# Patman86/SVT-AV1-Mod-by-Patman

Measured on AMD Instinct MI355X. Metric: encoded fps (4K 10-bit preset 8) + ME+txfm HBM GB/s vs roofline, 1/2/4/8 GPU, higher is better.
Workload: dtype u8 (ME) / int32 (transform)

## Files before the change

include/svt_hip_me.h:

```cpp
#ifndef SVT_HIP_ME_H
#define SVT_HIP_ME_H

#include "svt_hip.h"

#ifdef __cplusplus
extern "C" {
#endif

SVT_HIP_API void svt_sad_loop_kernel_hip(uint8_t *src, uint32_t src_stride, uint8_t *ref,
                                         uint32_t ref_stride, uint32_t block_height,
                                         uint32_t block_width, uint64_t *best_sad,
                                         int16_t *x_search_center, int16_t *y_search_center,
                                         uint32_t src_stride_raw, uint8_t skip_search_line,
                                         int16_t search_area_width, int16_t search_area_height);

SVT_HIP_API uint32_t svt_nxm_sad_kernel_hip(const uint8_t *src, uint32_t src_stride,
                                            const uint8_t *ref, uint32_t ref_stride,
                                            uint32_t height, uint32_t width);

SVT_HIP_API uint32_t svt_nxm_sad_kernel_sub_sampled_hip(const uint8_t *src, uint32_t src_stride,
                                                        const uint8_t *ref, uint32_t ref_stride,
                                                        uint32_t height, uint32_t width);
SVT_HIP_API uint32_t svt_aom_sad_16b_kernel_hip(uint16_t *src, uint32_t src_stride, uint16_t *ref,
                                                uint32_t ref_stride, uint32_t height, uint32_t width);
// ... 147 lines not shown
    uint64_t hme_sad;
    int16_t  hme_sc_x, hme_sc_y;
    uint8_t  do_ref;
    uint8_t  pad_[3];
} SvtHipMeSearchResult;

typedef struct SvtHipMeFrameOut {
    uint32_t *best_sad;
    uint32_t *best_mv;
    SvtHipMeSearchResult *search_results;
    uint32_t *me_mv_array;
    uint8_t  *me_candidate_array;
    uint8_t  *total_me_candidate_index;
    uint32_t *me_64x64_distortion, *me_32x32_distortion, *me_16x16_distortion, *me_8x8_distortion;
    uint32_t *me_8x8_cost_variance;
    uint32_t *rc_me_distortion;
} SvtHipMeFrameOut;

typedef struct SvtHipMeFrameJob {
    SvtHipMeParams   prm;
    SvtHipPyramid8   src;
    SvtHipPyramid8   ref[SVT_HIP_ME_MAX_LIST][SVT_HIP_ME_MAX_REF];
    SvtHipMeFrameOut out;
} SvtHipMeFrameJob;

SVT_HIP_API uint32_t svt_hip_me_b64_count(uint32_t width, uint32_t height);

SVT_HIP_API int32_t svt_hip_me_frames(const SvtHipMeFrameJob *jobs, uint32_t n_jobs, void *stream);

SVT_HIP_API int32_t svt_hip_me_validate_jobs(const SvtHipMeFrameJob *jobs, uint32_t n_jobs, uint32_t *max_b64);
SVT_HIP_API int32_t svt_hip_me_frames_dev(const SvtHipMeFrameJob *d_jobs, uint32_t n_jobs, uint32_t max_b64,
                                          void *stream);

typedef enum SvtHipRtcdSlot {
    SVT_HIP_SLOT_SAD_LOOP_KERNEL = 0,
    SVT_HIP_SLOT_NXM_SAD_KERNEL,
    SVT_HIP_SLOT_EXT_ALL_SAD_8X8_16X16,
    SVT_HIP_SLOT_EXT_EIGHT_SAD_32X32_64X64,
    SVT_HIP_SLOT_EXT_SAD_8X8_16X16,
    SVT_HIP_SLOT_EXT_SAD_32X32_64X64,
    SVT_HIP_SLOT_DOWNSAMPLE_2D,
    SVT_HIP_SLOT_COMPUTE_INTERM_VAR_FOUR8X8,
    SVT_HIP_SLOT_COMPUTE_SUB_MEAN_8X8,
    SVT_HIP_SLOT_COMPUTE_MEAN_8X8,
    SVT_HIP_SLOT_COMPUTE_MEAN_SQUARE_VALUES_8X8,
    SVT_HIP_SLOT_ME_COUNT
} SvtHipRtcdSlot;
SVT_HIP_API int32_t svt_hip_install_rtcd_me(void **table, uint32_t n_slots);

#ifdef __cplusplus
}
#endif
#endif
```

svt-av1-mod-by-patman_amd/csrc/me_frame.hip:

```cpp
#include <cstdio>
#include <cstdlib>
#include <cstring>

#include "common.hpp"
#include "sad_device.hpp"

using namespace svthip;
using namespace svthip::dev;

namespace {

#define NL 2
#define NR 4
#define MAX_SAD_VALUE_ (128 * 128 * 255)
#define MAX_U32_ 0xFFFFFFFFu

constexpr uint32_t ME_HME_WIN_DW = 3200;
constexpr uint32_t ME_WIN_DW     = ME_HME_WIN_DW - 64 * 16 - 256;
constexpr uint32_t fp_pitch_c(uint32_t tw) { return (((tw + 3) >> 2) + 17) | 1u; }
constexpr uint32_t FP_TILE_W = ME_WIN_DW / fp_pitch_c(64) >= 63 + 8 ? 64 : 32;
static_assert(ME_WIN_DW / fp_pitch_c(FP_TILE_W) >= 63 + 8, "full-pel window buffer too small for one tile");

struct PreHme {
    uint64_t sad;
    uint16_t sa_w, sa_h;
    int16_t  col, row;
    uint8_t  valid, pad_[7];
};

struct B64State {
    uint32_t org_x, org_y, b64_w, b64_h;
    SvtHipMeSearchResult sr[NL][NR];
    uint32_t reduce_div[NL][NR];
    uint32_t zz_sad[NL][NR];
    PreHme   ph[NL][NR][2];
    uint8_t  performed_phme[NL][NR][2];
    int16_t  l0x[NL][NR][2][2], l0y[NL][NR][2][2], l1x[NL][NR][2][2], l1y[NL][NR][2][2], l2x[NL][NR][2][2],
        l2y[NL][NR][2][2];
    uint64_t l0s[NL][NR][2][2], l1s[NL][NR][2][2], l2s[NL][NR][2][2];
    SvtHipSearchArea l0_min, l0_max;
    uint32_t wg_sum;
    int16_t  xc, yc, sw, sh, ox, oy;
    int32_t  do_centre, need_zero_sad, need_hme_sad;
    int16_t  stx, sty, stw, sth;
    int32_t  staged, restage;
    uint32_t zero_sad, hme_mv_sad;
    int16_t  fp_xc[NL * NR], fp_yc[NL * NR], fp_sw[NL * NR], fp_sh[NL * NR], fp_ox[NL * NR], fp_oy[NL * NR];
    uint8_t  fp_centre[NL * NR];
    uint32_t fp_inv[NL * NR];
    uint32_t first_ref_sad64;
    uint64_t me_sad_sum[NL][NR];
};

struct MeLds {
    static constexpr uint32_t WIN_DW = ME_WIN_DW, HME_WIN_DW = ME_HME_WIN_DW;
    SearchShared sh;
    B64State     st;
    union {
        alignas(16) uint32_t win[ME_HME_WIN_DW];
        struct {
            alignas(16) uint32_t fp_win_[ME_WIN_DW];
            alignas(16) uint32_t src_full[64 * 16];
            uint64_t bestkey[85];
            uint32_t me_dist[85];
        };
    };
    alignas(16) uint32_t src_q[32 * 8];
    alignas(16) uint32_t src_s[16 * 4];
};
static_assert(sizeof(MeLds::win) >= (ME_WIN_DW + 64 * 16) * 4 + 85 * 12, "full-pel view must fit the HME window buffer");

typedef __attribute__((address_space(1))) uint32_t g_u32;
#define MINV(a, b) ((a) < (b) ? (a) : (b))
#define MAXV(a, b) ((a) > (b) ? (a) : (b))
#define ABSV(a) ((a) < 0 ? -(a) : (a))

__device__ __forceinline__ uint32_t div_small(uint32_t x, uint32_t d) {
    return (d & (d - 1u)) == 0u && d ? x >> (31u - (uint32_t)__builtin_clz(d)) : x / d;
}

__device__ __forceinline__ uint16_t scaled_dist(uint16_t dist) {
    return (uint16_t)(((dist * 5) / 8) + ((dist % 8) == 0 ? 0 : 1));
}
__device__ __forceinline__ uint16_t pic_dist(const SvtHipMeParams &p, int li, int ri) {
    const int64_t d = (int64_t)p.picture_number - (int64_t)p.ref_picture_number[li][ri];
    return (uint16_t)(int16_t)ABSV(d);
}
__device__ __forceinline__ const uint8_t *plane_at(const SvtHipPlane8 &pl, int x, int y) {
    return pl.buf + (ptrdiff_t)((int)pl.org_y + y) * (ptrdiff_t)pl.stride + (int)pl.org_x + x;
}
__device__ __forceinline__ uint32_t load_u32_unaligned(const uint8_t *g) { return load_u32_any(g); }

__device__ __forceinline__ uint32_t block_sad16(const uint32_t *src, const uint8_t *ref, uint32_t ref_stride, uint32_t ndw, uint32_t rows,
                                                uint32_t row_step, uint32_t lane, uint32_t nlanes) {
    const uint32_t nch = (ndw + 3) >> 2, inv = make_inv_small(nch);
    uint32_t       acc = 0;
    for (uint32_t idx = lane; idx < nch * rows; idx += nlanes) {
        const uint32_t r = fast_div(idx, inv), ch = idx - r * nch;
        const uint4    sv = *(const uint4 *)&src[(r * row_step) * 16 + 4 * ch];
        const u128v    v  = load_u128_any(ref + (size_t)sad_mul_u24(r * row_step, ref_stride) + 16 * ch);
        const uint32_t nd = ndw - 4 * ch;
        acc = __builtin_amdgcn_sad_u8(sv.x, v.x, acc);
        acc = __builtin_amdgcn_sad_u8(sv.y, v.y, acc);
        if (nd > 2) {
            acc = __builtin_amdgcn_sad_u8(sv.z, v.z, acc);
            acc = __builtin_amdgcn_sad_u8(sv.w, v.w, acc);
        }
    }
    return acc;
}

template <class LDS>
__device__ void wg_block_sad(LDS &L, const uint8_t *ref, uint32_t ref_stride, uint32_t width, uint32_t rows,
                             uint32_t row_step) {
    if (threadIdx.x == 0)
        L.st.wg_sum = 0;
    __syncthreads();
    uint32_t acc = block_sad16(L.src_full, ref, ref_stride, width >> 2, rows, row_step, threadIdx.x, blockDim.x);
    acc = wave_sum(acc);
    if ((threadIdx.x & 63) == 0)
// ... 286 lines not shown
    if (use)
        total[pu] = off;
}

#ifdef SVT_HIP_ME_PROFILE
__device__ unsigned long long g_me_prof[16];
#define ME_SITE(k)             \
    do {                       \
        if (threadIdx.x == 0)  \
            L.sh.prof_site = k; \
    } while (0)
#define ME_PHASE(i)                                                        \
    do {                                                                   \
        if (threadIdx.x == 0) {                                            \
            const unsigned long long t_ = wall_clock64();                  \
            atomicAdd(&g_me_prof[i], t_ - prof_last);                      \
            prof_last = t_;                                                \
        }                                                                  \
    } while (0)
#else
#define ME_PHASE(i) \
    do {            \
    } while (0)
#define ME_SITE(k) \
    do {           \
    } while (0)
#endif


struct Ctx {
    const SvtHipMeFrameJob *job;
    uint32_t  b64, org_x, org_y, b64_w, b64_h, aw, ah;
    bool      hme_sub, me_sub;
    int       tl, nlists, R0, R1, nref;
};
__device__ __forceinline__ uint32_t opaque_v(uint32_t v) {
    asm volatile("" : "+v"(v));
    return v;
}
__device__ __forceinline__ uint32_t opaque_s(uint32_t v) {
    asm volatile("" : "+s"(v));
    return v;
}
#define ME_CTX_LOCALS(c)                                                                                                      \
    const SvtHipMeFrameJob &job = *(c).job;                                                                                   \
    const SvtHipMeParams   &p   = job.prm;                                                                                    \
    B64State               &S   = L.st;                                                                                       \
    const uint32_t tid = opaque_v(threadIdx.x), org_x = opaque_s((c).org_x), org_y = opaque_s((c).org_y);                       \
    const uint32_t b64_w = opaque_s((c).b64_w), b64_h = opaque_s((c).b64_h);                                                    \
    const uint32_t aw = (c).aw, ah = (c).ah;                                                                                  \
    const bool     hme_sub = (c).hme_sub, me_sub = (c).me_sub;                                                                \
    const int      tl = (c).tl, nlists = (c).nlists, R0 = (c).R0, R1 = (c).R1, nref = (c).nref;                               \
     \
    g_u32 *const gs = (g_u32 *)(job.out.best_sad + (size_t)(c).b64 * NL * NR * 85), *const gm = (g_u32 *)(job.out.best_mv + (size_t)(c).b64 * NL * NR * 85); \
    (void)job, (void)p, (void)S, (void)tid, (void)org_x, (void)org_y, (void)b64_w, (void)b64_h, (void)aw, (void)ah;           \
    (void)hme_sub, (void)me_sub, (void)tl, (void)nlists, (void)R0, (void)R1, (void)nref, (void)gs, (void)gm

__device__ bool make_ctx(Ctx &c, const SvtHipMeFrameJob &job, uint32_t bx) {
    const SvtHipMeParams &p = job.prm;
    c.job = &job;
    c.aw = (job.src.full.width + 7u) & ~7u, c.ah = (job.src.full.height + 7u) & ~7u;
    const uint32_t bw64 = (c.aw + 63) / 64, bh64 = (c.ah + 63) / 64;
    const uint32_t nb64 = bw64 * bh64, band = (nb64 + 7) / 8;
    c.b64 = (bx & 7) * band + (bx >> 3);
    if ((bx >> 3) >= band || c.b64 >= nb64)
        return false;
// ... 104 lines not shown
        const uint32_t best = slots_min((q.searched && (tl > 0 || q.li == 0)) ? z : MAX_U32_);
        if (q.searched && q.ri >= 1) {
            bool drop = tl > 0 && best < p.zz_sad_th && (uint32_t)((z - best) * 100u) > (uint32_t)(p.zz_sad_pct * best);
            if (p.me_safe_limit_zz_th)
                drop = drop || (p.hierarchical_levels > 0 && nlists == 2 && tl >= p.hierarchical_levels && p.similar_brightness_refs &&
                                S.zz_sad[0][0] < p.me_safe_limit_zz_th && S.zz_sad[1][0] < p.me_safe_limit_zz_th);
            if (drop)
                S.sr[q.li][q.ri].do_ref = 0;
        }
    }
}

struct SearchArgs {
    bool            search;
    uint32_t        nd;
    const uint32_t *src;
    uint32_t        row_dw, bw, bh, cap;
};

template <class LDS>
__device__ void prehme_round(LDS &L, const Ctx &c, int f0, int f1, bool searching, int part, SearchArgs &a) {
    ME_CTX_LOCALS(c);
    const int      f  = f0 + (int)(tid >> 1), si = (int)(tid & 1);
    const int      li = f < R0 ? 0 : 1, ri = f < R0 ? f : f - R0;
    const uint32_t nd = 2u * (uint32_t)(f1 - f0);
    const bool     mine = tid < nd;
    if (part == 0 && mine) {
        PreHme     &d  = S.ph[li][ri][si];
        SearchDesc &sd = L.sh.desc[tid];
        sd.aux_go      = 0;
        const SvtHipPlane8 &rp = job.ref[li][ri].sixteenth;
        sd.sa_w = sd.sa_h = 0, sd.skip = 0, sd.ref = rp.buf, sd.ref_stride = sd.raw_stride = rp.stride;
        if (tl > 0 || li == 0) {
            const uint32_t factor = scaled_dist(pic_dist(p, li, ri));
            const PreHme   o      = S.ph[0][ri][si];
            if (p.me_early_exit_th && S.zz_sad[li][ri] < p.me_early_exit_th) {
                d.col = d.row = 0, d.sad = 0, d.valid = 1;
            } else if (p.prehme_l1_early_exit && li == 1 && o.valid &&
                       ((o.sad < (32 * 32)) || ((ABSV(o.col) < 16) && (ABSV(o.row) < 16)))) {
                d.col = (int16_t)-o.col, d.row = (int16_t)-o.row, d.sad = o.sad, d.valid = 1;
            } else if (!S.sr[li][ri].do_ref) {
                d.col = d.row = 0, d.sad = MAX_U32_;
            } else {
                d.sa_w = (uint16_t)MINV((uint32_t)(p.prehme_sa_min[si].width * factor), (uint32_t)p.prehme_sa_max[si].width);
                d.sa_h = (uint16_t)MINV((uint32_t)(p.prehme_sa_min[si].height * factor), (uint32_t)p.prehme_sa_max[si].height);
                const int16_t ox16 = (int16_t)(((int16_t)org_x) >> 2), oy16 = (int16_t)(((int16_t)org_y) >> 2);
                int16_t pad_w = (int16_t)rp.org_x - 1, pad_h = (int16_t)rp.org_y - 1;
                int16_t sa_w = (int16_t)d.sa_w, sa_h = (int16_t)d.sa_h;
                int16_t ox = -(int16_t)(sa_w >> 1), oy = -(int16_t)(sa_h >> 1);
                const int16_t W = (int16_t)rp.width, H = (int16_t)rp.height;
                ox   = ((ox16 + ox) < -pad_w) ? (int16_t)(-pad_w - ox16) : ox;
                sa_w = ((ox16 + ox) < -pad_w) ? (int16_t)(sa_w - (-pad_w - (ox16 + ox))) : sa_w;
                ox   = ((ox16 + ox) > W - 1) ? (int16_t)(ox - ((ox16 + ox) - (W - 1))) : ox;
                sa_w = ((ox16 + ox + sa_w) > W) ? (int16_t)MAXV(1, sa_w - ((ox16 + ox + sa_w) - W)) : sa_w;
                oy   = ((oy16 + oy) < -pad_h) ? (int16_t)(-pad_h - oy16) : oy;
                sa_h = ((oy16 + oy) < -pad_h) ? (int16_t)(sa_h - (-pad_h - (oy16 + oy))) : sa_h;
                oy   = ((oy16 + oy) > H - 1) ? (int16_t)(oy - ((oy16 + oy) - (H - 1))) : oy;
                sa_h = ((oy16 + oy + sa_h) > H) ? (int16_t)MAXV(1, sa_h - ((oy16 + oy + sa_h) - H)) : sa_h;
                const int16_t x_tl = (int16_t)(((int16_t)rp.org_x + ox16) + ox);
                const int16_t y_tl = (int16_t)(((int16_t)rp.org_y + oy16) + oy);
                const uint32_t bw = b64_w >> 2, bh = hme_sub ? (b64_h >> 2) >> 1 : (b64_h >> 2);
                set_desc(sd, p, rp, x_tl, y_tl, sa_w, sa_h, p.prehme_skip_search_line && bw == 16 && bh <= 16);
                sd.aux_x = ox, sd.aux_y = oy, sd.aux_go = 1;
                S.performed_phme[li][ri][si] = 1;
            }
        } else {
            d.col = (int16_t)-S.ph[0][ri][si].col;
            d.row = (int16_t)-S.ph[0][ri][si].row;
            d.sad = S.ph[0][ri][si].sad;
        }
    }
    if (part == 0) {
        a = SearchArgs{searching, nd, L.src_s, hme_sub ? 8u : 4u, b64_w >> 2, hme_sub ? (b64_h >> 2) >> 1 : (b64_h >> 2), LDS::HME_WIN_DW};
        return;
    }
    if (searching) {
        if (mine && L.sh.desc[tid].aux_go) {
            PreHme       &d    = S.ph[li][ri][si];
            const int16_t q_ox = L.sh.desc[tid].aux_x, q_oy = L.sh.desc[tid].aux_y;
            decode_result(L.sh, tid, hme_sub, &d.sad, &d.col, &d.row);
            d.col = (int16_t)(d.col + q_ox);
            d.col = (int16_t)(d.col * 4);
            d.row = (int16_t)(d.row + q_oy);
            d.row = (int16_t)(d.row * 4);
            d.valid = 1;
        }
    }
    __syncthreads();
}

template <class LDS>
__device__ void phme_prune_lane0(LDS &L, const Ctx &c) {
    ME_CTX_LOCALS(c);
    if (tid < 64) {
        const Slot     q    = slot_of(tid, p, nlists);
        const uint32_t sad  = (uint32_t)MINV(S.ph[q.li][q.ri][0].sad, S.ph[q.li][q.ri][1].sad);
        const uint32_t best = slots_min((q.searched && (tl > 0 || q.li == 0)) ? sad : MAX_U32_);
        if (tl > 0 && best < p.phme_sad_th && q.searched && q.ri != 0 && S.sr[q.li][q.ri].do_ref &&
            (uint32_t)((sad - best) * 100u) > (uint32_t)(p.phme_sad_pct * best))
            S.sr[q.li][q.ri].do_ref = 0;
    }
}

template <class LDS>
__device__ void hme_l0_round(LDS &L, const Ctx &c, int f0, int f1, int part, SearchArgs &a) {
    ME_CTX_LOCALS(c);
// ... 572 lines not shown
            const uint64_t ssq = (uint64_t)lo + ((uint64_t)mid << 16) + ((uint64_t)hi << 32) + ((uint64_t)top << 48);
            const uint32_t d64 = L.me_dist[0];
            const uint32_t pix = b64_w * b64_h;
            out.me_8x8_cost_variance[b64] = (uint32_t)(ssq / 64);
            out.rc_me_distortion[b64]     = p.input_resolution_le_480p ? d8 : d16;
            out.me_64x64_distortion[b64]  = div_small(d64 * 4096u, pix);
            out.me_32x32_distortion[b64]  = div_small(d32 * 4096u, pix);
            out.me_16x16_distortion[b64]  = div_small(d16 * 4096u, pix);
            out.me_8x8_distortion[b64]    = div_small(d8 * 4096u, pix);
        }
    }
    if (tid < NL * NR)
        out.search_results[(size_t)b64 * NL * NR + tid] = (&S.sr[0][0])[tid];
}


#ifdef SVT_HIP_ME_ABLATE
__device__ int g_me_stop = 99;
#define ME_STOP(k)          \
    do {                    \
        if (me_stop == (k)) \
            return;         \
    } while (0)
#else
#define ME_STOP(k) \
    do {           \
    } while (0)
#endif

#ifndef SVT_HIP_ME_WGS
#define SVT_HIP_ME_WGS 8
#endif
template <bool MCTF>
__global__ __launch_bounds__(WG_THREADS, SVT_HIP_ME_WGS) void me_b64_kernel(const SvtHipMeFrameJob *__restrict__ jobs) {
    __shared__ MeLds L;
#ifdef SVT_HIP_ME_PROFILE
    unsigned long long prof_last = wall_clock64();
#endif
    __shared__ SvtHipMeFrameJob sjob;
    for (uint32_t i = threadIdx.x; i < sizeof(SvtHipMeFrameJob) / 4; i += blockDim.x)
        ((uint32_t *)&sjob)[i] = ((const uint32_t *)&jobs[blockIdx.y])[i];
    __syncthreads();
    Ctx c;
    if (!make_ctx(c, sjob, blockIdx.x))
        return;
#ifdef SVT_HIP_ME_ABLATE
    const int me_stop = g_me_stop;
#endif
    ME_CTX_LOCALS(c);
    stage_sources(L, c, 7);
    for (uint32_t i = tid; i < NL * NR * 85; i += blockDim.x) gs[i] = 0, gm[i] = 0;
    init_state_lane0(L, c);
    __syncthreads();
    ME_PHASE(0);
    ME_STOP(0);
    if (p.me_early_exit_th || p.me_safe_limit_zz_th) {
        zz_sad_all(L, c);
        zz_prune_lane0(L, c);
        __syncthreads();
    }
    ME_PHASE(1);
    ME_STOP(1);
    {
        const bool pre = p.prehme_enable, split = nlists == 2 && (p.prehme_l1_early_exit || tl == 0);
        const bool l0 = p.enable_hme_flag && p.enable_hme_level0_flag, l1 = p.enable_hme_flag && p.enable_hme_level1_flag;
        const bool l2 = p.enable_hme_flag && p.enable_hme_level2_flag;
        const bool dep = p.enable_me_sr_adjustment && p.distance_based_hme_resizing && p.reduce_hme_l0_sr_th_min &&
            p.reduce_hme_l0_sr_th_max && nref > 1;
        for (int step = 0; step < 6; step++) {
            if (step == 2) {
                if (pre) {
                    phme_prune_lane0(L, c);
                    __syncthreads();
                }
                ME_PHASE(2);
                ME_STOP(2);
            } else if (step == 4) {
                ME_PHASE(3);
                ME_STOP(3);
            } else if (step == 5) {
                ME_PHASE(4);
                ME_STOP(4);
                if (pre || l0 || l1) {
// ... 137 lines not shown
                return bad("reference planes need >= 64 samples of padding");
            if (!pyramid_ok(y))
                return bad("reference pyramid: decimated planes must be width>>1 / width>>2 with >= 32 / 16 samples of padding and stride >= width + 2 * org_x");
        }
    const void *outs[] = {j.out.best_sad, j.out.best_mv, j.out.search_results, j.out.me_mv_array, j.out.me_candidate_array,
                          j.out.total_me_candidate_index, j.out.me_64x64_distortion, j.out.me_32x32_distortion,
                          j.out.me_16x16_distortion, j.out.me_8x8_distortion, j.out.me_8x8_cost_variance,
                          j.out.rc_me_distortion};
    for (const void *o : outs)
        if (!o)
            return bad("NULL output array");
    return SVT_HIP_OK;
}

extern "C" int32_t svt_hip_me_validate_jobs(const SvtHipMeFrameJob *jobs, uint32_t n_jobs, uint32_t *max_b64_out) {
    if (!jobs || n_jobs == 0 || n_jobs > 65535) {
        set_error("svt_hip_me_frames: bad job count");
        return SVT_HIP_ERR_BAD_PARAMETER;
    }
    uint32_t max_b64 = 0;
    for (uint32_t i = 0; i < n_jobs; i++) {
        const int32_t rc = validate_job(jobs[i], i);
        if (rc != SVT_HIP_OK)
            return rc;
        const uint32_t nb = svt_hip_me_b64_count(jobs[i].src.full.width, jobs[i].src.full.height);
        max_b64           = nb > max_b64 ? nb : max_b64;
    }
    if (max_b64_out)
        *max_b64_out = max_b64;
    return SVT_HIP_OK;
}

static void launch_me(const SvtHipMeFrameJob *d_jobs, uint32_t n_jobs, uint32_t max_b64, hipStream_t st, bool mctf) {
    if (mctf)
        hipLaunchKernelGGL(me_b64_kernel<true>, dim3((max_b64 + 7) / 8 * 8, n_jobs), dim3(WG_THREADS), 0, st, d_jobs);
    else
        hipLaunchKernelGGL(me_b64_kernel<false>, dim3((max_b64 + 7) / 8 * 8, n_jobs), dim3(WG_THREADS), 0, st, d_jobs);
}

extern "C" int32_t svt_hip_me_frames_dev(const SvtHipMeFrameJob *d_jobs, uint32_t n_jobs, uint32_t max_b64, void *stream) {
    if (!d_jobs || n_jobs == 0 || n_jobs > 65535 || max_b64 == 0) {
        set_error("svt_hip_me_frames_dev: bad argument");
        return SVT_HIP_ERR_BAD_PARAMETER;
    }
    if (!ensure_init())
        return SVT_HIP_ERR_NO_DEVICE;
    launch_me(d_jobs, n_jobs, max_b64, resolve_stream(stream), false);
    SVT_HIP_CHECK(hipGetLastError());
    return SVT_HIP_OK;
}

extern "C" int32_t svt_hip_me_frames(const SvtHipMeFrameJob *jobs, uint32_t n_jobs, void *stream) {
    uint32_t      max_b64 = 0;
    const int32_t vrc     = svt_hip_me_validate_jobs(jobs, n_jobs, &max_b64);
    if (vrc != SVT_HIP_OK)
        return vrc;
    TierBCall c("svt_hip_me_frames", stream);
    const SvtHipMeFrameJob *d_jobs = (const SvtHipMeFrameJob *)c.stage(jobs, sizeof(SvtHipMeFrameJob) * n_jobs);
    if (!d_jobs)
        return c.status();
    bool mctf = true;
    for (uint32_t i = 0; i < n_jobs; i++) mctf = mctf && jobs[i].prm.me_mctf;
    launch_me(d_jobs, n_jobs, max_b64, c.stream(), mctf);
    return c.finish();
}

extern "C" int32_t svt_hip_install_rtcd_me(void **table, uint32_t n_slots) {
    if (!table || n_slots < SVT_HIP_SLOT_ME_COUNT) {
        set_error("svt_hip_install_rtcd_me: table too small");
        return SVT_HIP_ERR_BAD_PARAMETER;
// ... 24 lines not shown
```

svt-av1-mod-by-patman_amd/svtav1_hip/prototypes.py:

```python
PROTOTYPES = {
    "svt_aom_cdef_find_dir_dual_hip": (None, ("c_void_p", "c_void_p", "c_int", "c_void_p", "c_void_p", "c_int32", "c_void_p", "c_void_p")),
    "svt_aom_cdef_find_dir_hip": ("c_uint8", ("c_void_p", "c_int32", "c_void_p", "c_int32")),
    "svt_aom_copy_rect8_8bit_to_16bit_hip": (None, ("c_void_p", "c_int32", "c_void_p", "c_int32", "c_int32", "c_int32")),
    "svt_aom_downsample_2d_hip": (None, ("c_void_p", "c_uint32", "c_uint32", "c_uint32", "c_void_p", "c_uint32", "c_uint32")),
    "svt_aom_highbd_lpf_horizontal_14_hip": (None, ("c_void_p", "c_int32", "c_void_p", "c_void_p", "c_void_p", "c_int32")),
    "svt_aom_highbd_lpf_horizontal_4_hip": (None, ("c_void_p", "c_int32", "c_void_p", "c_void_p", "c_void_p", "c_int32")),
    "svt_aom_highbd_lpf_horizontal_6_hip": (None, ("c_void_p", "c_int32", "c_void_p", "c_void_p", "c_void_p", "c_int32")),
    "svt_aom_highbd_lpf_horizontal_8_hip": (None, ("c_void_p", "c_int32", "c_void_p", "c_void_p", "c_void_p", "c_int32")),
    "svt_aom_highbd_lpf_vertical_14_hip": (None, ("c_void_p", "c_int32", "c_void_p", "c_void_p", "c_void_p", "c_int32")),
    "svt_aom_highbd_lpf_vertical_4_hip": (None, ("c_void_p", "c_int32", "c_void_p", "c_void_p", "c_void_p", "c_int32")),
    "svt_aom_highbd_lpf_vertical_6_hip": (None, ("c_void_p", "c_int32", "c_void_p", "c_void_p", "c_void_p", "c_int32")),
    "svt_aom_highbd_lpf_vertical_8_hip": (None, ("c_void_p", "c_int32", "c_void_p", "c_void_p", "c_void_p", "c_int32")),
    "svt_aom_highbd_quantize_b_hip": (None, ("c_void_p", "c_ssize_t", "c_void_p", "c_void_p", "c_void_p", "c_void_p", "c_void_p", "c_void_p", "c_void_p", "c_void_p", "c_void_p", "c_void_p", "c_void_p", "c_void_p", "c_int32")),
    "svt_aom_highbd_subtract_block_hip": (None, ("c_int", "c_int", "c_void_p", "c_ssize_t", "c_void_p", "c_ssize_t", "c_void_p", "c_ssize_t", "c_int")),
    "svt_aom_lpf_horizontal_14_hip": (None, ("c_void_p", "c_int32", "c_void_p", "c_void_p", "c_void_p")),
    "svt_aom_lpf_horizontal_4_hip": (None, ("c_void_p", "c_int32", "c_void_p", "c_void_p", "c_void_p")),
    "svt_aom_lpf_horizontal_6_hip": (None, ("c_void_p", "c_int32", "c_void_p", "c_void_p", "c_void_p")),
    "svt_aom_lpf_horizontal_8_hip": (None, ("c_void_p", "c_int32", "c_void_p", "c_void_p", "c_void_p")),
    "svt_aom_lpf_vertical_14_hip": (None, ("c_void_p", "c_int32", "c_void_p", "c_void_p", "c_void_p")),
    "svt_aom_lpf_vertical_4_hip": (None, ("c_void_p", "c_int32", "c_void_p", "c_void_p", "c_void_p")),
    "svt_aom_lpf_vertical_6_hip": (None, ("c_void_p", "c_int32", "c_void_p", "c_void_p", "c_void_p")),
    "svt_aom_lpf_vertical_8_hip": (None, ("c_void_p", "c_int32", "c_void_p", "c_void_p", "c_void_p")),
    "svt_aom_quantize_b_hip": (None, ("c_void_p", "c_ssize_t", "c_void_p", "c_void_p", "c_void_p", "c_void_p", "c_void_p", "c_void_p", "c_void_p", "c_void_p", "c_void_p", "c_void_p", "c_void_p", "c_void_p", "c_int32")),
    "svt_aom_sad_16b_kernel_hip": ("c_uint32", ("c_void_p", "c_uint32", "c_void_p", "c_uint32", "c_uint32", "c_uint32")),
# ... 136 lines not shown
    "svt_handle_transform64x64_N2_N4_hip": ("c_uint64", ("c_void_p",)),
    "svt_handle_transform64x64_hip": ("c_uint64", ("c_void_p",)),
    "svt_hip_analysis_frames": ("c_int32", ("c_void_p", "c_uint32", "c_int32", "c_int32", "c_void_p")),
    "svt_hip_blend_batch": ("c_int32", ("c_void_p", "c_uint32", "c_void_p")),
    "svt_hip_cdef_apply_frame": ("c_int32", ("c_void_p", "c_uint32", "c_void_p", "c_void_p", "c_int32", "c_int32", "c_void_p", "c_void_p", "c_void_p")),
    "svt_hip_cdef_apply_plane": ("c_int32", ("c_void_p", "c_void_p", "c_void_p", "c_int32", "c_int32", "c_void_p", "c_void_p", "c_void_p")),
    "svt_hip_cdef_search_plane": ("c_int32", ("c_void_p", "c_void_p", "c_void_p", "c_void_p", "c_void_p", "c_void_p", "c_void_p")),
    "svt_hip_comm_create": ("c_int32", ("c_void_p", "c_int32", "c_int32", "c_void_p")),
    "svt_hip_comm_destroy": ("c_int32", ("c_void_p",)),
    "svt_hip_comm_get_unique_id": ("c_int32", ("c_void_p",)),
    "svt_hip_compound_mask_search_batch": ("c_int32", ("c_void_p", "c_void_p", "c_uint32", "c_void_p")),
    "svt_hip_convolve_batch": ("c_int32", ("c_void_p", "c_uint32", "c_void_p")),
    "svt_hip_convolve_sr_batch": ("c_int32", ("c_void_p", "c_uint32", "c_void_p")),
    "svt_hip_copy": ("c_int32", ("c_void_p", "c_void_p", "c_size_t", "c_void_p")),
    "svt_hip_debug_inject_failure": (None, ("c_int32",)),
    "svt_hip_debug_tier_a_broken": ("c_int32", ("c_int32",)),
    "svt_hip_device_count": ("c_int32", ()),
    "svt_hip_download": ("c_int32", ("c_void_p", "c_void_p", "c_size_t", "c_void_p")),
    "svt_hip_download_2d": ("c_int32", ("c_void_p", "c_size_t", "c_void_p", "c_size_t", "c_size_t", "c_size_t", "c_void_p")),
    "svt_hip_event_destroy": ("c_int32", ("c_void_p",)),
    "svt_hip_free": ("c_int32", ("c_void_p",)),
    "svt_hip_host_alloc": ("c_int32", ("c_void_p", "c_size_t")),
    "svt_hip_host_free": ("c_int32", ("c_void_p",)),
    "svt_hip_init": ("c_int32", ("c_int32",)),
    "svt_hip_install_rtcd": ("c_int32", ("c_void_p", "c_uint32", "c_void_p")),
    "svt_hip_install_rtcd_me": ("c_int32", ("c_void_p", "c_uint32")),
    "svt_hip_intra_search_frames": ("c_int32", ("c_void_p", "c_uint32", "c_void_p")),
    "svt_hip_last_error": ("c_char_p", ()),
    "svt_hip_loop_filter_frame": ("c_int32", ("c_void_p", "c_void_p")),
    "svt_hip_malloc": ("c_int32", ("c_void_p", "c_size_t")),
    "svt_hip_me_b64_count": ("c_uint32", ("c_uint32", "c_uint32")),
    "svt_hip_me_frames": ("c_int32", ("c_void_p", "c_uint32", "c_void_p")),
    "svt_hip_me_frames_dev": ("c_int32", ("c_void_p", "c_uint32", "c_uint32", "c_void_p")),
    "svt_hip_me_validate_jobs": ("c_int32", ("c_void_p", "c_uint32", "c_void_p")),
    "svt_hip_memset": ("c_int32", ("c_void_p", "c_int", "c_size_t", "c_void_p")),
    "svt_hip_pad_plane": ("c_int32", ("c_void_p", "c_void_p")),
    "svt_hip_plane_sse": ("c_int32", ("c_void_p", "c_uint32", "c_void_p", "c_uint32", "c_uint32", "c_uint32", "c_int32", "c_void_p", "c_void_p")),
    "svt_hip_publish_reference": ("c_int32", ("c_void_p", "c_size_t", "c_int32", "c_void_p", "c_void_p", "c_void_p", "c_void_p")),
    "svt_hip_pyramid_frame": ("c_int32", ("c_void_p", "c_void_p", "c_void_p", "c_int32", "c_void_p")),
    "svt_hip_quantize_batch": ("c_int32", ("c_void_p", "c_void_p", "c_void_p", "c_uint32", "c_uint32", "c_void_p")),
    "svt_hip_restoration_filter_frame": ("c_int32", ("c_void_p", "c_uint32", "c_void_p")),
    "svt_hip_rtcd_lookup": ("c_void_p", ("c_char_p",)),
    "svt_hip_sad_loop_batch": ("c_int32", ("c_void_p", "c_void_p", "c_void_p", "c_uint32", "c_void_p")),
    "svt_hip_sgr_apply_unit": ("c_int32", ("c_void_p", "c_int32", "c_void_p", "c_void_p", "c_uint32", "c_void_p")),
    "svt_hip_sgr_filter_unit": ("c_int32", ("c_void_p", "c_int32", "c_void_p", "c_void_p", "c_uint32", "c_void_p")),
    "svt_hip_sgr_search_unit": ("c_int32", ("c_void_p", "c_int32", "c_int32", "c_int32", "c_int32", "c_void_p", "c_void_p", "c_void_p", "c_void_p")),
    "svt_hip_sgr_search_work_bytes": ("c_size_t", ("c_uint32", "c_uint32", "c_int32")),
    "svt_hip_shard_layer": ("c_uint32", ("c_uint32", "c_uint32")),
    "svt_hip_shard_owner": ("c_uint32", ("c_uint32", "c_uint32", "c_uint32")),
    "svt_hip_shard_owner_gop": ("c_uint32", ("c_uint64", "c_uint32", "c_uint32")),
    "svt_hip_shard_segment": (None, ("c_uint32", "c_uint32", "c_uint32", "c_uint32", "c_uint32", "c_void_p")),
    "svt_hip_shard_slot": ("c_uint32", ("c_uint32", "c_uint32")),
    "svt_hip_shutdown": (None, ()),
    "svt_hip_stream_create": ("c_int32", ("c_void_p",)),
    "svt_hip_stream_destroy": ("c_int32", ("c_void_p",)),
    "svt_hip_stream_sync": ("c_int32", ("c_void_p",)),
    "svt_hip_tf_accumulate_batch": ("c_int32", ("c_void_p", "c_uint32", "c_void_p")),
    "svt_hip_tf_central_batch": ("c_int32", ("c_void_p", "c_uint32", "c_void_p")),
    "svt_hip_tf_estimate_noise": ("c_int32", ("c_void_p", "c_uint32", "c_uint32", "c_uint32", "c_int32", "c_int32", "c_void_p", "c_void_p")),
    "svt_hip_tf_filter_blocks": ("c_int32", ("c_void_p", "c_uint32", "c_void_p", "c_void_p", "c_uint32", "c_uint32", "c_uint32", "c_void_p")),
    "svt_hip_tf_filter_picture": ("c_int32", ("c_void_p", "c_void_p")),
    "svt_hip_tf_normalise_batch": ("c_int32", ("c_void_p", "c_void_p", "c_uint32", "c_void_p")),
    "svt_hip_tf_workspace_bytes": ("c_uint64", ("c_uint32", "c_uint32", "c_uint32")),
    "svt_hip_tf_workspace_state_offset": ("c_uint64", ("c_uint32", "c_uint32", "c_uint32", "c_uint32")),
    "svt_hip_tier_a_failed_over": ("c_int32", ()),
    "svt_hip_tpl_dispenser_frame": ("c_int32", ("c_void_p", "c_void_p")),
# ... 22 lines not shown
```

Measured before the change: 5438.

## Move pre-HME search into a picture-wide kernel sharing reference windows across B64 rows

Adds a separate pre-HME kernel that processes whole rows or columns of 64x64 blocks at once. It stages one shared sixteenth-resolution reference window in LDS for many neighbouring blocks and writes the best SAD and MV per block into the output buffer as records. The main ME kernel then loads these records and skips the inline pre-HME search when every entry is served. This is meant to cut redundant reference loads and per-block search latency, at the cost of an extra launch, more code, and reuse of the output buffer and the unused search-key LDS as scratch. It is on by default and can be turned off with an environment variable.

After: 5346. -1.7%, worse.

```diff
diff --git a/include/svt_hip_me.h b/include/svt_hip_me.h
--- a/include/svt_hip_me.h
+++ b/include/svt_hip_me.h
@@ -203,6 +203,10 @@
 SVT_HIP_API int32_t svt_hip_me_frames_dev(const SvtHipMeFrameJob *d_jobs, uint32_t n_jobs, uint32_t max_b64,
                                           void *stream);
 
+SVT_HIP_API int32_t svt_hip_me_set_prehme_kernel(int32_t on);
+SVT_HIP_API int32_t svt_hip_me_prehme_dev(const SvtHipMeFrameJob *d_jobs, uint32_t n_jobs, uint32_t max_b64,
+                                          void *stream);
+
 typedef enum SvtHipRtcdSlot {
     SVT_HIP_SLOT_SAD_LOOP_KERNEL = 0,
     SVT_HIP_SLOT_NXM_SAD_KERNEL,
diff --git a/svt-av1-mod-by-patman_amd/csrc/me_frame.hip b/svt-av1-mod-by-patman_amd/csrc/me_frame.hip
--- a/svt-av1-mod-by-patman_amd/csrc/me_frame.hip
+++ b/svt-av1-mod-by-patman_amd/csrc/me_frame.hip
@@ -3,6 +3,7 @@
 #include <cstring>
 
 #include "common.hpp"
+#include "me_prehme.hpp"
 #include "sad_device.hpp"
 
 using namespace svthip;
@@ -68,6 +69,8 @@
     alignas(16) uint32_t src_q[32 * 8];
     alignas(16) uint32_t src_s[16 * 4];
 };
+static_assert(2 * NL * NR <= MAX_SEARCH / 2 && (MAX_SEARCH / 2) * sizeof(uint64_t) >= PREHME_REC_DW * 4, "pre-HME records do not fit the unused search keys");
+template <class LDS> __device__ __forceinline__ uint32_t *ph_rec(LDS &L) { return (uint32_t *)&L.sh.best[MAX_SEARCH / 2]; }
 static_assert(sizeof(MeLds::win) >= (ME_WIN_DW + 64 * 16) * 4 + 85 * 12, "full-pel view must fit the HME window buffer");
 
 typedef __attribute__((address_space(1))) uint32_t g_u32;
@@ -79,13 +82,6 @@
     return (d & (d - 1u)) == 0u && d ? x >> (31u - (uint32_t)__builtin_clz(d)) : x / d;
 }
 
-__device__ __forceinline__ uint16_t scaled_dist(uint16_t dist) {
-    return (uint16_t)(((dist * 5) / 8) + ((dist % 8) == 0 ? 0 : 1));
-}
-__device__ __forceinline__ uint16_t pic_dist(const SvtHipMeParams &p, int li, int ri) {
-    const int64_t d = (int64_t)p.picture_number - (int64_t)p.ref_picture_number[li][ri];
-    return (uint16_t)(int16_t)ABSV(d);
-}
 __device__ __forceinline__ const uint8_t *plane_at(const SvtHipPlane8 &pl, int x, int y) {
     return pl.buf + (ptrdiff_t)((int)pl.org_y + y) * (ptrdiff_t)pl.stride + (int)pl.org_x + x;
 }
@@ -438,6 +434,7 @@
     const SvtHipMeFrameJob *job;
     uint32_t  b64, org_x, org_y, b64_w, b64_h, aw, ah;
     bool      hme_sub, me_sub;
+    bool      rec;
     int       tl, nlists, R0, R1, nref;
 };
 __device__ __forceinline__ uint32_t opaque_v(uint32_t v) {
@@ -608,7 +605,6 @@
         const SvtHipPlane8 &rp = job.ref[li][ri].sixteenth;
         sd.sa_w = sd.sa_h = 0, sd.skip = 0, sd.ref = rp.buf, sd.ref_stride = sd.raw_stride = rp.stride;
         if (tl > 0 || li == 0) {
-            const uint32_t factor = scaled_dist(pic_dist(p, li, ri));
             const PreHme   o      = S.ph[0][ri][si];
             if (p.me_early_exit_th && S.zz_sad[li][ri] < p.me_early_exit_th) {
                 d.col = d.row = 0, d.sad = 0, d.valid = 1;
@@ -618,26 +614,16 @@
             } else if (!S.sr[li][ri].do_ref) {
                 d.col = d.row = 0, d.sad = MAX_U32_;
             } else {
-                d.sa_w = (uint16_t)MINV((uint32_t)(p.prehme_sa_min[si].width * factor), (uint32_t)p.prehme_sa_max[si].width);
-                d.sa_h = (uint16_t)MINV((uint32_t)(p.prehme_sa_min[si].height * factor), (uint32_t)p.prehme_sa_max[si].height);
-                const int16_t ox16 = (int16_t)(((int16_t)org_x) >> 2), oy16 = (int16_t)(((int16_t)org_y) >> 2);
-                int16_t pad_w = (int16_t)rp.org_x - 1, pad_h = (int16_t)rp.org_y - 1;
-                int16_t sa_w = (int16_t)d.sa_w, sa_h = (int16_t)d.sa_h;
-                int16_t ox = -(int16_t)(sa_w >> 1), oy = -(int16_t)(sa_h >> 1);
-                const int16_t W = (int16_t)rp.width, H = (int16_t)rp.height;
-                ox   = ((ox16 + ox) < -pad_w) ? (int16_t)(-pad_w - ox16) : ox;
-                sa_w = ((ox16 + ox) < -pad_w) ? (int16_t)(sa_w - (-pad_w - (ox16 + ox))) : sa_w;
-                ox   = ((ox16 + ox) > W - 1) ? (int16_t)(ox - ((ox16 + ox) - (W - 1))) : ox;
-                sa_w = ((ox16 + ox + sa_w) > W) ? (int16_t)MAXV(1, sa_w - ((ox16 + ox + sa_w) - W)) : sa_w;
-                oy   = ((oy16 + oy) < -pad_h) ? (int16_t)(-pad_h - oy16) : oy;
-                sa_h = ((oy16 + oy) < -pad_h) ? (int16_t)(sa_h - (-pad_h - (oy16 + oy))) : sa_h;
-                oy   = ((oy16 + oy) > H - 1) ? (int16_t)(oy - ((oy16 + oy) - (H - 1))) : oy;
-                sa_h = ((oy16 + oy + sa_h) > H) ? (int16_t)MAXV(1, sa_h - ((oy16 + oy + sa_h) - H)) : sa_h;
-                const int16_t x_tl = (int16_t)(((int16_t)rp.org_x + ox16) + ox);
-                const int16_t y_tl = (int16_t)(((int16_t)rp.org_y + oy16) + oy);
-                const uint32_t bw = b64_w >> 2, bh = hme_sub ? (b64_h >> 2) >> 1 : (b64_h >> 2);
-                set_desc(sd, p, rp, x_tl, y_tl, sa_w, sa_h, p.prehme_skip_search_line && bw == 16 && bh <= 16);
-                sd.aux_x = ox, sd.aux_y = oy, sd.aux_go = 1;
+                const uint32_t rec_mv = c.rec ? ph_rec(L)[2 * PREHME_REC_ENTRY(li, ri, si) + 1] : PREHME_REC_NONE;
+                const PrehmeArea ar = prehme_area(job, li, ri, si, org_x, org_y, b64_w, b64_h);
+                d.sa_w = ar.sa_w0, d.sa_h = ar.sa_h0;
+                if (rec_mv != PREHME_REC_NONE) {
+                    d.sad = ph_rec(L)[2 * PREHME_REC_ENTRY(li, ri, si)];
+                    d.col = (int16_t)(rec_mv & 0xffffu), d.row = (int16_t)(rec_mv >> 16), d.valid = 1;
+                } else {
+                    set_desc(sd, p, rp, ar.x_tl, ar.y_tl, ar.sa_w, ar.sa_h, p.prehme_skip_search_line && ar.bw == 16 && ar.bh <= 16);
+                    sd.aux_x = ar.ox, sd.aux_y = ar.oy, sd.aux_go = 1;
+                }
                 S.performed_phme[li][ri][si] = 1;
             }
         } else {
@@ -647,7 +633,17 @@
         }
     }
     if (part == 0) {
-        a = SearchArgs{searching, nd, L.src_s, hme_sub ? 8u : 4u, b64_w >> 2, hme_sub ? (b64_h >> 2) >> 1 : (b64_h >> 2), LDS::HME_WIN_DW};
+        bool search = searching;
+        if (c.rec) {
+            if (tid < 64) {
+                const uint64_t go = __ballot(mine && L.sh.desc[tid].aux_go);
+                if (tid == 0)
+                    S.wg_sum = go != 0;
+            }
+            __syncthreads();
+            search = searching && S.wg_sum;
+        }
+        a = SearchArgs{search, nd, L.src_s, hme_sub ? 8u : 4u, b64_w >> 2, hme_sub ? (b64_h >> 2) >> 1 : (b64_h >> 2), LDS::HME_WIN_DW};
         return;
     }
     if (searching) {
@@ -1286,7 +1282,7 @@
 #define SVT_HIP_ME_WGS 8
 #endif
 template <bool MCTF>
-__global__ __launch_bounds__(WG_THREADS, SVT_HIP_ME_WGS) void me_b64_kernel(const SvtHipMeFrameJob *__restrict__ jobs) {
+__global__ __launch_bounds__(WG_THREADS, SVT_HIP_ME_WGS) void me_b64_kernel(const SvtHipMeFrameJob *__restrict__ jobs, uint32_t have_records) {
     __shared__ MeLds L;
 #ifdef SVT_HIP_ME_PROFILE
     unsigned long long prof_last = wall_clock64();
@@ -1301,8 +1297,11 @@
 #ifdef SVT_HIP_ME_ABLATE
     const int me_stop = g_me_stop;
 #endif
+    c.rec = have_records != 0;
     ME_CTX_LOCALS(c);
     stage_sources(L, c, 7);
+    if (c.rec && tid < PREHME_REC_DW)
+        ph_rec(L)[tid] = gs[tid];
     for (uint32_t i = tid; i < NL * NR * 85; i += blockDim.x) gs[i] = 0, gm[i] = 0;
     init_state_lane0(L, c);
     __syncthreads();
@@ -1506,10 +1505,14 @@
 }
 
 static void launch_me(const SvtHipMeFrameJob *d_jobs, uint32_t n_jobs, uint32_t max_b64, hipStream_t st, bool mctf) {
-    if (mctf)
-        hipLaunchKernelGGL(me_b64_kernel<true>, dim3((max_b64 + 7) / 8 * 8, n_jobs), dim3(WG_THREADS), 0, st, d_jobs);
-    else
-        hipLaunchKernelGGL(me_b64_kernel<false>, dim3((max_b64 + 7) / 8 * 8, n_jobs), dim3(WG_THREADS), 0, st, d_jobs);
+    if (mctf) {
+        hipLaunchKernelGGL(me_b64_kernel<true>, dim3((max_b64 + 7) / 8 * 8, n_jobs), dim3(WG_THREADS), 0, st, d_jobs, 0u);
+        return;
+    }
+    const bool pre = prehme_kernel_enabled();
+    if (pre)
+        launch_prehme_picture(d_jobs, n_jobs, st);
+    hipLaunchKernelGGL(me_b64_kernel<false>, dim3((max_b64 + 7) / 8 * 8, n_jobs), dim3(WG_THREADS), 0, st, d_jobs, pre ? 1u : 0u);
 }
 
 extern "C" int32_t svt_hip_me_frames_dev(const SvtHipMeFrameJob *d_jobs, uint32_t n_jobs, uint32_t max_b64, void *stream) {
diff --git a/svt-av1-mod-by-patman_amd/csrc/me_prehme.hip b/svt-av1-mod-by-patman_amd/csrc/me_prehme.hip
--- /dev/null
+++ b/svt-av1-mod-by-patman_amd/csrc/me_prehme.hip
@@ -0,0 +1,256 @@
+#include <atomic>
+#include <cstdlib>
+#include <cstring>
+
+#include "common.hpp"
+#include "me_prehme.hpp"
+#include "sad_device.hpp"
+
+using namespace svthip;
+using namespace svthip::dev;
+
+namespace {
+
+constexpr uint32_t PH_WIN_DW  = 6144;
+constexpr uint32_t PH_SRC_DW  = 2048;
+constexpr uint32_t PH_PIECE   = 64;
+constexpr uint32_t PH_MAX_N   = 4096;
+constexpr uint32_t PH_WGS     = 4;
+constexpr uint32_t B64_OUT_DW = SVT_HIP_ME_MAX_LIST * SVT_HIP_ME_MAX_REF * SVT_HIP_ME_SQUARE_PUS;
+
+struct PhB64 {
+    uint32_t woff;
+    int16_t  sa_w, sa_h, ox, oy;
+    uint32_t best;
+};
+struct PhLds {
+    alignas(16) uint32_t win[PH_WIN_DW + 8];
+    alignas(16) uint32_t src[PH_SRC_DW];
+    PhB64    b[PH_PIECE];
+    uint32_t npiece, pitch, nrows;
+    int32_t  xmin, ymin;
+};
+
+typedef __attribute__((address_space(1))) uint32_t g_u32;
+
+struct PhJob {
+    uint32_t bw64, nb64, nfx, nfy;
+    uint32_t nserved;
+    uint32_t nmark;
+    uint32_t units;
+};
+__device__ __forceinline__ PhJob ph_job(const SvtHipMeFrameJob &job) {
+    const SvtHipMeParams &p = job.prm;
+    PhJob                 g;
+    const uint32_t aw = (job.src.full.width + 7u) & ~7u, ah = (job.src.full.height + 7u) & ~7u;
+    g.bw64 = (aw + 63) / 64, g.nb64 = g.bw64 * ((ah + 63) / 64);
+    g.nfx = aw / 64, g.nfy = ah / 64;
+    const uint32_t R0 = p.num_of_ref_pic_to_search[0], R1 = p.num_of_list_to_search > 1 ? p.num_of_ref_pic_to_search[1] : 0;
+    g.nserved = (p.prehme_enable && !p.prehme_skip_search_line) ? (p.temporal_layer_index > 0 ? R0 + R1 : R0) : 0u;
+    g.nmark   = (g.nb64 * PREHME_REC_DW + 255u) / 256u;
+    g.units   = g.nmark + g.nserved * (g.nfx + g.nfy);
+    return g;
+}
+
+template <int CTRL> __device__ __forceinline__ uint32_t dpp_min(uint32_t v) {
+    return min(v, (uint32_t)__builtin_amdgcn_update_dpp((int)v, (int)v, CTRL, 0xf, 0xf, false));
+}
+__device__ __forceinline__ uint32_t wave_min_all(uint32_t v) {
+    v = dpp_min<0xB1>(v);
+    v = dpp_min<0x4E>(v);
+    v = dpp_min<0x124>(v);
+    v = dpp_min<0x128>(v);
+    v = min(v, (uint32_t)__shfl_xor((int)v, 16, 64));
+    v = min(v, (uint32_t)__shfl_xor((int)v, 32, 64));
+    return v;
+}
+
+__device__ __forceinline__ void put_record(const SvtHipMeFrameJob &job, uint32_t b64, uint32_t entry, uint32_t sad, uint32_t mv) {
+    g_u32 *o = (g_u32 *)(job.out.best_sad + (size_t)b64 * B64_OUT_DW) + 2 * entry;
+    o[0] = sad, o[1] = mv;
+}
+
+template <bool SUB>
+__device__ void ph_unit(PhLds &L, const SvtHipMeFrameJob &job, const PhJob &g, int li, int ri, int si, uint32_t s) {
+    constexpr uint32_t BH = SUB ? 8 : 16, KK = SUB ? 2 : 1, RPP = (BH - 1) * KK + 1;
+    constexpr uint32_t CAP = PH_SRC_DW / (BH * 4) < PH_PIECE ? PH_SRC_DW / (BH * 4) : PH_PIECE;
+    const uint32_t tid = threadIdx.x, lane = tid & 63u;
+    const uint32_t n     = si == 0 ? g.nfy : g.nfx;
+    const uint32_t entry = PREHME_REC_ENTRY(li, ri, si);
+    const SvtHipPlane8 &rp = job.ref[li][ri].sixteenth;
+    const PrehmeArea a0  = prehme_area(job, li, ri, si, 0, 0, 64, 64);
+    const uint32_t   no0 = ((((uint32_t)a0.sa_w0 + 3u) >> 2) + 1u) >> 1, N = (uint32_t)a0.sa_h0 * no0;
+    if (N == 0 || N > PH_MAX_N) {
+        for (uint32_t t = tid; t < n; t += blockDim.x)
+            put_record(job, si == 0 ? t * g.bw64 + s : s * g.bw64 + t, entry, 0, PREHME_REC_NONE);
+        return;
+    }
+    const uint32_t inv_n = make_inv(N), inv_no = make_inv_small(no0);
+    for (uint32_t b0 = 0; b0 < n;) {
+        if (tid < 64) {
+            const bool     in = tid < CAP && b0 + tid < n;
+            const uint32_t t  = in ? b0 + tid : b0;
+            const PrehmeArea a = prehme_area(job, li, ri, si, si == 0 ? s * 64 : t * 64, si == 0 ? t * 64 : s * 64, 64, 64);
+            const bool     bad = a.sa_w <= 0 || a.sa_h <= 0 || a.x_tl < 0 || a.y_tl < 0;
+            int32_t xlo = a.x_tl, ylo = a.y_tl;
+            int32_t xhi = a.x_tl + 4 * (int32_t)((((uint32_t)a.sa_w + 3u) >> 2) + 5u);
+            int32_t yhi = a.y_tl + a.sa_h - 1 + (int32_t)RPP;
+#pragma unroll
+            for (int off = 1; off < 64; off <<= 1) {
+                const int32_t x0 = __shfl_up(xlo, off, 64), y0 = __shfl_up(ylo, off, 64), x1 = __shfl_up(xhi, off, 64), y1 = __shfl_up(yhi, off, 64);
+                if ((int)tid >= off)
+                    xlo = min(xlo, x0), ylo = min(ylo, y0), xhi = max(xhi, x1), yhi = max(yhi, y1);
+            }
+            const int32_t  x_first = __shfl(a.x_tl, 0, 64);
+            const uint32_t pitch   = ((uint32_t)(xhi - xlo) >> 2) | 1u;
+            const bool     viol    = !in || bad || ((a.x_tl - x_first) & 3) != 0 || pitch * (uint32_t)(yhi - ylo) > PH_WIN_DW;
+            const uint64_t vm      = __ballot(viol);
+            const uint32_t np      = vm ? (uint32_t)__ffsll((unsigned long long)vm) - 1u : 64u;
+            const int last = np ? (int)np - 1 : 0;
+            const int32_t  bx0 = __shfl(xlo, last, 64), by0 = __shfl(ylo, last, 64);
+            const uint32_t bp = __shfl(pitch, last, 64), br = (uint32_t)(__shfl(yhi, last, 64) - by0);
+            if (tid < np) {
+                PhB64 &B = L.b[tid];
+                B.woff = (uint32_t)(a.y_tl - by0) * bp + ((uint32_t)(a.x_tl - bx0) >> 2);
+                B.sa_w = a.sa_w, B.sa_h = a.sa_h, B.ox = a.ox, B.oy = a.oy, B.best = ~0u;
+            }
+            if (tid == 0) {
+                L.npiece = np, L.pitch = bp, L.nrows = br, L.xmin = bx0, L.ymin = by0;
+                if (np == 0)
+                    put_record(job, si == 0 ? b0 * g.bw64 + s : s * g.bw64 + b0, entry, 0, PREHME_REC_NONE);
+            }
+        }
+        __syncthreads();
+        const uint32_t np = L.npiece, pitch = L.pitch;
+        if (np == 0) {
+            b0 += 1;
+            __syncthreads();
+            continue;
+        }
+        stage_rows16(L.win, pitch, rp.buf + (ptrdiff_t)L.ymin * (ptrdiff_t)rp.stride + L.xmin, rp.stride, L.nrows, blockDim.x, tid);
+        for (uint32_t idx = tid; idx < np * BH; idx += blockDim.x) {
+            const uint32_t k = idx / BH, r = idx % BH, t = b0 + k;
+            const uint32_t sx = (si == 0 ? s : t) * 16, sy = (si == 0 ? t : s) * 16 + r * KK;
+            const SvtHipPlane8 &sp = job.src.sixteenth;
+            const u128v v = load_u128_any(sp.buf + (ptrdiff_t)(sp.org_y + sy) * (ptrdiff_t)sp.stride + sp.org_x + sx);
+            *(uint4 *)&L.src[idx * 4] = make_uint4(v.x, v.y, v.z, v.w);
+        }
+        __syncthreads();
+        const uint32_t total = np * N;
+        for (uint32_t base = tid & ~63u; base < total; base += blockDim.x) {
+            const uint32_t i = base + lane, ic = i < total ? i : total - 1;
+            const uint32_t k = fast_div(ic, inv_n), l = ic - sad_mul_u24(k, N);
+            const uint32_t j = fast_div(l, inv_no), q = 2u * (l - sad_mul_u24(j, no0));
+            const PhB64    B = L.b[k];
+            uint32_t       key = ~0u;
+            if (i < total && j < (uint32_t)B.sa_h && 4 * q < (uint32_t)B.sa_w) {
+                uint32_t sad[8];
+                oct_sad_fixed<16>(&L.win[B.woff + sad_mul_u24(j, pitch) + q], KK * pitch, &L.src[k * BH * 4], 4, BH, sad);
+                const uint32_t nvalid = (uint32_t)B.sa_w - 4 * q;
+#pragma unroll
+                for (uint32_t p = 0; p < 8; p++)
+                    if (p < nvalid)
+                        key = min(key, (sad[p] << 16) | (l << 3) | p);
+            }
+            const uint32_t kf = __builtin_amdgcn_readfirstlane(k), kl = __builtin_amdgcn_readlane(k, 63);
+            for (uint32_t kk = kf; kk <= kl; kk++) {
+                const uint32_t v = wave_min_all(k == kk ? key : ~0u);
+                if (lane == 0 && v != ~0u)
+                    atomicMin(&L.b[kk].best, v);
+            }
+        }
+        __syncthreads();
+        if (tid < np) {
+            const PhB64    B   = L.b[tid];
+            const uint32_t t   = b0 + tid, b64 = si == 0 ? t * g.bw64 + s : s * g.bw64 + t;
+            if (B.best == ~0u) {
+                put_record(job, b64, entry, 0, PREHME_REC_NONE);
+            } else {
+                const uint32_t l = (B.best & 0xffffu) >> 3, p = B.best & 7u, j = fast_div(l, inv_no), col = 8u * (l - j * no0) + p;
+                const int16_t  x = (int16_t)((int16_t)((int16_t)col + B.ox) * 4), y = (int16_t)((int16_t)((int16_t)j + B.oy) * 4);
+                put_record(job, b64, entry, (B.best >> 16) * KK, (uint32_t)(uint16_t)x | ((uint32_t)(uint16_t)y << 16));
+            }
+        }
+        b0 += np;
+    }
+}
+
+__global__ __launch_bounds__(WG_THREADS, PH_WGS) void prehme_picture_kernel(const SvtHipMeFrameJob *__restrict__ jobs, uint32_t n_jobs) {
+    __shared__ PhLds            L;
+    __shared__ SvtHipMeFrameJob sjob;
+    const uint32_t tid = threadIdx.x;
+    uint32_t       off = 0;
+    for (uint32_t ji = 0; ji < n_jobs; ji++) {
+        const PhJob g = ph_job(jobs[ji]);
+        const uint32_t first = (blockIdx.x + gridDim.x - off) % gridDim.x;
+        off = (off + g.units) % gridDim.x;
+        if (first >= g.units)
+            continue;
+        __syncthreads();
+        for (uint32_t i = tid; i < sizeof(SvtHipMeFrameJob) / 4; i += blockDim.x) ((uint32_t *)&sjob)[i] = ((const uint32_t *)&jobs[ji])[i];
+        __syncthreads();
+        const SvtHipMeParams &p  = sjob.prm;
+        const uint32_t        R0 = p.num_of_ref_pic_to_search[0], nlists = p.num_of_list_to_search, tl = p.temporal_layer_index;
+        for (uint32_t u = first; u < g.units; u += gridDim.x) {
+            if (u < g.nmark) {
+                const uint32_t dw = u * 256u + tid, b64 = dw / PREHME_REC_DW, e = (dw % PREHME_REC_DW) >> 1;
+                const uint32_t li = e >> 3, ri = (e >> 1) & 3u;
+                const bool full   = (b64 % g.bw64) < g.nfx && (b64 / g.bw64) < g.nfy;
+                const bool served = g.nserved && full && li < nlists && ri < p.num_of_ref_pic_to_search[li] && (tl > 0 || li == 0);
+                if (b64 < g.nb64 && !served)
+                    ((g_u32 *)(sjob.out.best_sad + (size_t)b64 * B64_OUT_DW))[dw % PREHME_REC_DW] = (dw & 1u) ? PREHME_REC_NONE : 0u;
+                continue;
+            }
+            const uint32_t v = u - g.nmark, per = g.nfx + g.nfy, f = v / per, s = v - f * per;
+            const int      li = f < R0 ? 0 : 1, ri = (int)(f < R0 ? f : f - R0);
+            const int      si = s < g.nfx ? 0 : 1;
+            __syncthreads();
+            if (p.hme_search_method == 0)
+                ph_unit<true>(L, sjob, g, li, ri, si, si ? s - g.nfx : s);
+            else
+                ph_unit<false>(L, sjob, g, li, ri, si, si ? s - g.nfx : s);
+        }
+    }
+}
+
+std::atomic<int32_t> g_prehme_on{-1};
+int32_t prehme_setting() {
+    int32_t v = g_prehme_on.load(std::memory_order_relaxed);
+    if (v < 0) {
+        const char *e   = getenv("SVTAV1_HIP_ME_PREHME");
+        int32_t     def = (e && !strcmp(e, "inline")) ? 0 : 1, expect = -1;
+        g_prehme_on.compare_exchange_strong(expect, def);
+        v = g_prehme_on.load(std::memory_order_relaxed);
+    }
+    return v;
+}
+
+}
+
+namespace svthip {
+bool prehme_kernel_enabled() { return prehme_setting() != 0; }
+void launch_prehme_picture(const SvtHipMeFrameJob *d_jobs, uint32_t n_jobs, hipStream_t st) {
+    const int cus = cu_count();
+    hipLaunchKernelGGL(prehme_picture_kernel, dim3((uint32_t)(cus > 0 ? cus : 256) * PH_WGS), dim3(WG_THREADS), 0, st, d_jobs, n_jobs);
+}
+}
+
+extern "C" int32_t svt_hip_me_set_prehme_kernel(int32_t on) {
+    const int32_t prev = prehme_setting();
+    g_prehme_on.store(on ? 1 : 0, std::memory_order_relaxed);
+    return prev;
+}
+
+extern "C" int32_t svt_hip_me_prehme_dev(const SvtHipMeFrameJob *d_jobs, uint32_t n_jobs, uint32_t max_b64, void *stream) {
+    if (!d_jobs || n_jobs == 0 || n_jobs > 65535 || max_b64 == 0) {
+        set_error("svt_hip_me_prehme_dev: bad argument");
+        return SVT_HIP_ERR_BAD_PARAMETER;
+    }
+    if (!ensure_init())
+        return SVT_HIP_ERR_NO_DEVICE;
+    launch_prehme_picture(d_jobs, n_jobs, resolve_stream(stream));
+    SVT_HIP_CHECK(hipGetLastError());
+    return SVT_HIP_OK;
+}
+
+SVT_HIP_MODULE_WARMUP(me_prehme)
diff --git a/svt-av1-mod-by-patman_amd/csrc/me_prehme.hpp b/svt-av1-mod-by-patman_amd/csrc/me_prehme.hpp
--- /dev/null
+++ b/svt-av1-mod-by-patman_amd/csrc/me_prehme.hpp
@@ -0,0 +1,65 @@
+#pragma once
+
+#include <hip/hip_runtime.h>
+#include <stdint.h>
+
+#include "../../include/svt_hip_me.h"
+
+namespace svthip {
+
+constexpr uint32_t PREHME_REC_DW   = 32;
+constexpr uint32_t PREHME_REC_NONE = 0x7fff7fffu;
+#define PREHME_REC_ENTRY(li, ri, si) ((((li) * SVT_HIP_ME_MAX_REF + (ri)) << 1) | (si))
+
+void launch_prehme_picture(const SvtHipMeFrameJob *d_jobs, uint32_t n_jobs, hipStream_t st);
+bool prehme_kernel_enabled();
+
+namespace dev {
+
+__device__ __forceinline__ uint16_t scaled_dist(uint16_t dist) {
+    return (uint16_t)(((dist * 5) / 8) + ((dist % 8) == 0 ? 0 : 1));
+}
+__device__ __forceinline__ uint16_t pic_dist(const SvtHipMeParams &p, int li, int ri) {
+    const int64_t d = (int64_t)p.picture_number - (int64_t)p.ref_picture_number[li][ri];
+    return (uint16_t)(int16_t)(d < 0 ? -d : d);
+}
+
+struct PrehmeArea {
+    uint16_t sa_w0, sa_h0;
+    int16_t  sa_w, sa_h;
+    int16_t  ox, oy;
+    int32_t  x_tl, y_tl;
+    uint32_t bw, bh;
+};
+__device__ __forceinline__ PrehmeArea prehme_area(const SvtHipMeFrameJob &job, int li, int ri, int si, uint32_t org_x, uint32_t org_y,
+                                                  uint32_t b64_w, uint32_t b64_h) {
+    const SvtHipMeParams &p  = job.prm;
+    const SvtHipPlane8   &rp = job.ref[li][ri].sixteenth;
+    PrehmeArea            a;
+    const uint32_t factor = scaled_dist(pic_dist(p, li, ri));
+    const uint32_t w0 = (uint32_t)(p.prehme_sa_min[si].width * factor), h0 = (uint32_t)(p.prehme_sa_min[si].height * factor);
+    a.sa_w0 = (uint16_t)(w0 < (uint32_t)p.prehme_sa_max[si].width ? w0 : (uint32_t)p.prehme_sa_max[si].width);
+    a.sa_h0 = (uint16_t)(h0 < (uint32_t)p.prehme_sa_max[si].height ? h0 : (uint32_t)p.prehme_sa_max[si].height);
+    const int16_t ox16 = (int16_t)(((int16_t)org_x) >> 2), oy16 = (int16_t)(((int16_t)org_y) >> 2);
+    const int16_t pad_w = (int16_t)rp.org_x - 1, pad_h = (int16_t)rp.org_y - 1;
+    int16_t       sa_w = (int16_t)a.sa_w0, sa_h = (int16_t)a.sa_h0;
+    int16_t       ox = -(int16_t)(sa_w >> 1), oy = -(int16_t)(sa_h >> 1);
+    const int16_t W = (int16_t)rp.width, H = (int16_t)rp.height;
+    ox   = ((ox16 + ox) < -pad_w) ? (int16_t)(-pad_w - ox16) : ox;
+    sa_w = ((ox16 + ox) < -pad_w) ? (int16_t)(sa_w - (-pad_w - (ox16 + ox))) : sa_w;
+    ox   = ((ox16 + ox) > W - 1) ? (int16_t)(ox - ((ox16 + ox) - (W - 1))) : ox;
+    sa_w = ((ox16 + ox + sa_w) > W) ? (int16_t)((sa_w - ((ox16 + ox + sa_w) - W)) > 1 ? (sa_w - ((ox16 + ox + sa_w) - W)) : 1) : sa_w;
+    oy   = ((oy16 + oy) < -pad_h) ? (int16_t)(-pad_h - oy16) : oy;
+    sa_h = ((oy16 + oy) < -pad_h) ? (int16_t)(sa_h - (-pad_h - (oy16 + oy))) : sa_h;
+    oy   = ((oy16 + oy) > H - 1) ? (int16_t)(oy - ((oy16 + oy) - (H - 1))) : oy;
+    sa_h = ((oy16 + oy + sa_h) > H) ? (int16_t)((sa_h - ((oy16 + oy + sa_h) - H)) > 1 ? (sa_h - ((oy16 + oy + sa_h) - H)) : 1) : sa_h;
+    a.sa_w = sa_w, a.sa_h = sa_h, a.ox = ox, a.oy = oy;
+    a.x_tl = (int16_t)(((int16_t)rp.org_x + ox16) + ox);
+    a.y_tl = (int16_t)(((int16_t)rp.org_y + oy16) + oy);
+    a.bw   = b64_w >> 2;
+    a.bh   = p.hme_search_method == 0 ? (b64_h >> 2) >> 1 : (b64_h >> 2);
+    return a;
+}
+
+}
+}
diff --git a/svt-av1-mod-by-patman_amd/svtav1_hip/prototypes.py b/svt-av1-mod-by-patman_amd/svtav1_hip/prototypes.py
--- a/svt-av1-mod-by-patman_amd/svtav1_hip/prototypes.py
+++ b/svt-av1-mod-by-patman_amd/svtav1_hip/prototypes.py
@@ -192,6 +192,8 @@
     "svt_hip_me_b64_count": ("c_uint32", ("c_uint32", "c_uint32")),
     "svt_hip_me_frames": ("c_int32", ("c_void_p", "c_uint32", "c_void_p")),
     "svt_hip_me_frames_dev": ("c_int32", ("c_void_p", "c_uint32", "c_uint32", "c_void_p")),
+    "svt_hip_me_prehme_dev": ("c_int32", ("c_void_p", "c_uint32", "c_uint32", "c_void_p")),
+    "svt_hip_me_set_prehme_kernel": ("c_int32", ("c_int32",)),
     "svt_hip_me_validate_jobs": ("c_int32", ("c_void_p", "c_uint32", "c_void_p")),
     "svt_hip_memset": ("c_int32", ("c_void_p", "c_int", "c_size_t", "c_void_p")),
     "svt_hip_pad_plane": ("c_int32", ("c_void_p", "c_void_p")),
```
